# szhan227/text2protein

Measured on AMD Instinct MI355X. Metric: 6D backbone samples/sec (128-res, 1000-step), higher is better.
Workload: dtype f16; 1 GPU; cfg2: test_config.yml L=128 N=1000 chains/GPU=32 C=5 text_tokens=512 condition=none; step = 1 PC step (2 score evals + SDE updates); sample = 1000 PC steps; finite=True

## Files before the change

### include/t2p.h

```cpp
#ifndef T2P_H_
#define T2P_H_

#include <stdint.h>

#ifdef __cplusplus
extern "C" {
#endif

#define T2P_DTYPE_F32 0
#define T2P_DTYPE_BF16 1
#define T2P_DTYPE_F16 2

#define T2P_SDE_VE 0
#define T2P_SDE_VP 1

typedef struct t2p_model_config {
  int32_t num_channels;
  int32_t max_res_num;
  int32_t nf;
  int32_t num_res_blocks;
  int32_t n_ch_mult;
  int32_t ch_mult[8];
  int32_t n_attn_resolutions;
  int32_t attn_resolutions[8];
// ... 80 lines not shown
void t2p_train_destroy(t2p_trainer* t);
int t2p_train_num_params(const t2p_trainer* t);
int t2p_train_param_info(const t2p_trainer* t, int i, const char** name, int64_t shape[4], int* ndim);
int t2p_train_load_param(t2p_trainer* t, const char* name, const float* host_data, const int64_t* shape, int ndim);
int t2p_train_read(t2p_trainer* t, int which, const char* name, float* host_out);
int t2p_train_write(t2p_trainer* t, int which, const char* name, const float* host_in);
int t2p_train_set_step(t2p_trainer* t, int64_t step, int64_t adam_updates, int64_t ema_updates);
int t2p_train_get_step(const t2p_trainer* t, int64_t out3[3]);
int t2p_train_set_dropout_masks(t2p_trainer* t, const uint8_t* const* device_masks, int n);
int t2p_train_loss(t2p_trainer* t, const t2p_train_batch* batch, int backward, float* loss_host, float* score_out, void* stream);
int t2p_train_step(t2p_trainer* t, const t2p_train_batch* batch, float* loss_host, void* stream);
int t2p_train_grad_buffer(t2p_trainer* t, float** device_ptr, int64_t* n);
int t2p_train_apply(t2p_trainer* t, void* stream);
int t2p_train_eval_loss(t2p_trainer* t, const t2p_train_batch* batch, float* loss_host, void* stream);
int64_t t2p_train_device_bytes(const t2p_trainer* t);
int t2p_op_tgemm(const float* A, int64_t sAm, int64_t sAk, const float* B, int64_t sBk, int64_t sBn, float* C, int64_t ldc, int M, int N,
                 int K, int nz, int64_t sAz, int64_t sBz, int64_t sCz, float alpha, float beta, const float* bias_n, int ksplit, int conv,
                 int H, int W, int conv_C, void* stream);
int t2p_op_tgemm16(int dtype, const float* A, int64_t sAm, int64_t sAk, const float* B, int64_t sBk, int64_t sBn, float* C, int64_t ldc,
                   int M, int N, int K, int nz, int64_t sAz, int64_t sBz, int64_t sCz, float alpha, float beta, const float* bias_n, int ksplit,
                   int conv, int H, int W, int conv_C, void* stream);
int t2p_op_groupnorm_backward(const float* x, const float* dy, const float* gamma, const float* beta, int silu, int batch, int HW, int C,
                              int groups, float eps, float* dx, float* dgamma, float* dbeta, void* stream);
int t2p_op_layernorm_backward(const float* x, const float* dy, const float* gamma, int64_t rows, int C, float eps, float* dx, float* dgamma,
                              float* dbeta, void* stream);
int t2p_op_softmax_backward(const float* P, float* dP_inout, int64_t rows, int n, float scale, void* stream);
int t2p_op_geglu_backward(const float* u, const float* dy, float* du, int64_t rows, int inner, void* stream);

int t2p_op_gemm(int dtype, const void* A, int a_f32, const void* Bw, void* C, int c_f32, int M, int N, int K,
                int64_t lda, int64_t ldb, int64_t ldc, const float* bias_n, const float* residual, float alpha,
                void* stream);
int t2p_op_gemm_r16(int dtype, const void* A, int a_f32, const void* Bw, void* C, int c_f32, int M, int N, int K, int64_t lda,
                    int64_t ldb, int64_t ldc, const float* bias_n, const void* residual16, float alpha, void* stream);
int t2p_op_conv3x3(int dtype, const void* x, int a_f32, const void* w, const float* bias, float* out, int batch,
                   int H, int W, int Cin, int Cout, int upsample, void* stream);
int t2p_op_conv3x3_shortcut(int dtype, const void* a, const void* w, const float* bias, const void* x0, int CX0,
                            const void* x1, int CX1, float alpha, void* out, int c_f32, int batch, int H, int W, int C,
                            int Cout, void* stream);
int t2p_op_conv3x3_groupnorm(int dtype, const void* a, const void* w, const float* bias, const float* bias_bn, const void* residual,
                             float alpha, int upsample, int groups, const float* gamma, const float* beta, float eps, int silu,
                             void* out, int out_f32, void* normed, float* col_stats, int batch, int H, int W, int C, int Cout, void* stream);
int t2p_op_small_conv_groupnorm(int dtype, const void* a, const void* w, int64_t ldw, const void* x0, int CX0, const void* x1, int CX1,
                                const float* bias, const float* bias_bn, const void* residual, float alpha, void* out, int out_f32,
                                float* col_stats, void* normed, int groups, const float* gamma, const float* beta, float eps, int silu,
                                int batch, int H, int W, int C, int Cout, void* stream);
int t2p_op_st_entry(int dtype, const void* x, const float* col_stats, int groups, const float* gn_gamma, const float* gn_beta,
                    float gn_eps, const void* w_in, const float* b_in, const void* residual, const float* ln_gamma,
                    const float* ln_beta, float ln_eps, const void* w_2, int n2, const float* b_2, int geglu, void* t, void* out2,
                    const void* w_3, const float* b_3, const void* res3, void* y, float* y_stats, int batch, int n, int C,
                    void* stream);
int t2p_op_attn_proj(int dtype, const void* x, const float* col_stats, int groups, const float* gn_gamma, const float* gn_beta,
                     float gn_eps, const void* w_qk, const float* b_qk, const void* w_v, void* qk, void* vt, void* k_fm,
                     int64_t npad, int batch, int n, int C, void* stream);
int t2p_op_input_conv(const float* x, const float* w_tcn, const float* bias, void* out, int out_dtype, int batch, int C,
                      int H, int W, int nf, float* col_stats, void* stream);
int t2p_op_groupnorm(const float* x0, const float* x1, int C0, int C1, int batch, int H, int W, int groups,
                     const float* gamma, const float* beta, float eps, int silu, int down, void* out, int dtype,
                     void* stream);
int t2p_op_layernorm(const float* x, const float* gamma, const float* beta, void* out, int dtype, int64_t rows,
                     int C, float eps, void* stream);
int t2p_op_layernorm16(const void* x16, const float* gamma, const float* beta, void* out16, int dtype, int64_t rows, int C,
                       float eps, void* stream);
int t2p_op_softmax(const float* S, int64_t lds, void* P, int64_t ldp, int dtype, int64_t rows, int n, float scale,
                   void* stream);
int t2p_op_geglu(const float* u, void* out, int dtype, int64_t rows, int inner, void* stream);
int64_t t2p_op_attention_ws(int dtype, int batch, int heads, int nq, int nk);
// ... 47 lines not shown
```

### text2protein_amd/_lib.py

```python
from __future__ import annotations

import ctypes as C

from . import build as _build

DT_F32, DT_BF16, DT_F16 = 0, 1, 2
DTYPE_NAMES = {"f32": DT_F32, "fp32": DT_F32, "float32": DT_F32, "bf16": DT_BF16, "bfloat16": DT_BF16,
               "f16": DT_F16, "fp16": DT_F16, "float16": DT_F16}
SDE_VE, SDE_VP = 0, 1


class T2PError(RuntimeError):
    pass


class ModelConfig(C.Structure):
    _fields_ = [("num_channels", C.c_int32), ("max_res_num", C.c_int32), ("nf", C.c_int32),
                ("num_res_blocks", C.c_int32), ("n_ch_mult", C.c_int32), ("ch_mult", C.c_int32 * 8),
                ("n_attn_resolutions", C.c_int32), ("attn_resolutions", C.c_int32 * 8),
                ("n_heads", C.c_int32), ("context_dim", C.c_int32), ("num_scales", C.c_int32),
                ("sigma_min", C.c_double), ("sigma_max", C.c_double),
                ("skip_rescale", C.c_int32), ("scale_by_sigma", C.c_int32), ("compute_dtype", C.c_int32)]


# ... 28 lines not shown
    "t2p_engine_load_param": (_i, [_vp, C.c_char_p, _vp, C.POINTER(_i64), _i]),
    "t2p_engine_finalize": (_i, [_vp]),
    "t2p_engine_set_context": (_i, [_vp, _vp, _i, _i, _vp]),
    "t2p_engine_score": (_i, [_vp, _vp, _vp, _vp, _i, _vp]),
    "t2p_engine_score_ex": (_i, [_vp, _vp, _vp, _vp, _vp, _i, _vp]),
    "t2p_engine_device_bytes": (_i64, [_vp]),
    "t2p_engine_pool_reclaimed": (_i, [_vp]),
    "t2p_sampler_create": (_i, [_vp, C.POINTER(SamplerConfig), _vp, _vp, C.POINTER(_vp)]),
    "t2p_sampler_set_seed": (_i, [_vp, _u64]),
    "t2p_sampler_set_norm_allreduce": (_i, [_vp, _vp, _vp, _vp]),
    "t2p_built_with_ablation": (_i, []),
    "t2p_sampler_destroy": (None, [_vp]),
    "t2p_sampler_set_condition": (_i, [_vp, _vp, _vp]),
    "t2p_sampler_reset": (_i, [_vp, _i, _vp]),
    "t2p_sampler_step": (_i, [_vp, _vp, _vp, _vp, _vp, _vp]),
    "t2p_sampler_step_graph": (_i, [_vp, _vp, _vp, _vp]),
    "t2p_sampler_run": (_i, [_vp, _vp, _vp, _i, _i, _vp]),
    "t2p_sampler_set_vp_tables": (_i, [_vp, _vp, _vp, _vp, _vp]),
    "t2p_sampler_count_dispatches": (_i, [_vp, _vp, _vp, _vp, C.POINTER(C.c_int)]),
    "t2p_op_gemm": (_i, [_i, _vp, _i, _vp, _vp, _i, _i, _i, _i, _i64, _i64, _i64, _vp, _vp, _f, _vp]),
    "t2p_op_conv3x3_shortcut": (_i, [_i, _vp, _vp, _vp, _vp, _i, _vp, _i, _f, _vp, _i, _i, _i, _i, _i, _i, _vp]),
    "t2p_op_conv3x3_groupnorm": (_i, [_i, _vp, _vp, _vp, _vp, _vp, C.c_float, _i, _i, _vp, _vp, C.c_float, _i, _vp, _i, _vp, _vp,
                                      _i, _i, _i, _i, _i, _vp]),
    "t2p_op_attention_wide": (_i, [_i, _vp, _i64, _vp, _i64, _vp, _i64, _vp, _i, _vp, _vp, _i, _f, _vp, _i, _i, _i, _f, _vp]),
    "t2p_op_attention_wide_fm": (_i, [_i, _vp, _i64, _vp, _vp, _vp, _i, _vp, _vp, _i, _f, _vp, _i, _i, _i, _f, _vp]),
    "t2p_op_gemm_frag_major": (_i, [_i, _vp, _vp, _vp, _vp, _i, _i, _i, _i, _i, _i, _vp]),
    "t2p_op_small_conv_groupnorm": (_i, [_i, _vp, _vp, _i64, _vp, _i, _vp, _i, _vp, _vp, _vp, _f, _vp, _i, _vp, _vp, _i, _vp, _vp, _f, _i,
                                         _i, _i, _i, _i, _i, _vp]),
    "t2p_op_attn_proj": (_i, [_i, _vp, _vp, _i, _vp, _vp, _f, _vp, _vp, _vp, _vp, _vp, _vp, _i64, _i, _i, _i, _vp]),
    "t2p_op_st_entry": (_i, [_i, _vp, _vp, _i, _vp, _vp, _f, _vp, _vp, _vp, _vp, _vp, _f, _vp, _i, _vp, _i, _vp, _vp, _vp, _vp, _vp, _vp, _vp,
                             _i, _i, _i, _vp]),
    "t2p_op_input_conv": (_i, [_vp, _vp, _vp, _vp, _i, _i, _i, _i, _i, _i, _vp, _vp]),
    "t2p_op_gemm_r16": (_i, [_i, _vp, _i, _vp, _vp, _i, _i, _i, _i, _i64, _i64, _i64, _vp, _vp, _f, _vp]),
    "t2p_op_conv3x3": (_i, [_i, _vp, _i, _vp, _vp, _vp, _i, _i, _i, _i, _i, _i, _vp]),
    "t2p_op_groupnorm": (_i, [_vp, _vp, _i, _i, _i, _i, _i, _i, _vp, _vp, _f, _i, _i, _vp, _i, _vp]),
    "t2p_op_layernorm": (_i, [_vp, _vp, _vp, _vp, _i, _i64, _i, _f, _vp]),
    "t2p_op_layernorm16": (_i, [_vp, _vp, _vp, _vp, _i, _i64, _i, _f, _vp]),
    "t2p_op_softmax": (_i, [_vp, _i64, _vp, _i64, _i, _i64, _i, _f, _vp]),
    "t2p_op_geglu": (_i, [_vp, _vp, _i, _i64, _i, _vp]),
    "t2p_op_attention_ws": (_i64, [_i, _i, _i, _i, _i]),
    "t2p_op_attention_qkv": (_i, [_i, _vp, _i64, _vp, _i, _i, _i, _i, _f, _vp]),
    "t2p_op_attention": (_i, [_i, _vp, _i64, _vp, _i64, _vp, _i64, _vp, _i, _i, _i, _i, _i, _f, _vp, _vp]),
    "t2p_op_langevin": (_i, [_vp, _vp, _vp, _vp, _vp, _vp, _vp, _i, _i64, _f, _f, _vp, _vp]),
    "t2p_op_langevin_norms": (_i, [_vp, _vp, _i, _i64, _vp, _vp, _vp]),
    "t2p_op_langevin_update": (_i, [_vp, _vp, _vp, _vp, _vp, _vp, _vp, _i64, _vp, _f, _f, _f, _vp]),
    "t2p_op_apply_mask": (_i, [_vp, _vp, _vp, _i64, _vp]),
    "t2p_op_predictor": (_i, [_vp, _vp, _vp, _vp, _vp, _vp, _vp, _i64, _f, _i, _vp]),
    "t2p_op_philox_normal": (_i, [_vp, _i64, _u64, _u64, _vp]),
    "t2p_profile_begin": (_i, []),
    "t2p_debug_set": (_i, [_i, _i]),
    "t2p_op_decode_6d": (_i, [_vp, _i, _i, _i, _vp, _vp, _vp, _vp]),
    "t2p_op_embedding_gather": (_i, [_vp, _i, _vp, _vp, _i64, _i, _i, _vp, _vp]),
    "t2p_profile_end": (_i, [C.POINTER(C.c_double)]),
    "t2p_profile_dominant": (_i, [C.POINTER(C.c_double), C.c_char_p, C.c_int]),
    "t2p_profile_attention": (_i, [C.POINTER(C.c_double)]),
    "t2p_profile_shapes": (_i, [C.c_char_p, C.c_int]),
    "t2p_debug_tap": (_i, [_i, _vp, C.c_int64, C.POINTER(C.c_int64)]),
    "t2p_profile_layers_begin": (_i, []),
    "t2p_profile_layers_end": (_i, [C.c_char_p, C.c_int]),
    "t2p_op_convert": (_i, [_vp, _vp, _i, _i64, _vp]),
    "t2p_train_create": (_i, [C.POINTER(ModelConfig), C.POINTER(TrainConfig), C.POINTER(_vp)]),
    "t2p_train_destroy": (None, [_vp]),
    "t2p_train_num_params": (_i, [_vp]),
    "t2p_train_param_info": (_i, [_vp, _i, C.POINTER(C.c_char_p), C.POINTER(_i64), C.POINTER(_i)]),
    "t2p_train_load_param": (_i, [_vp, C.c_char_p, _vp, C.POINTER(_i64), _i]),
    "t2p_train_read": (_i, [_vp, _i, C.c_char_p, _vp]),
# ... 102 lines not shown
```

### text2protein_amd/build.py

```python
from __future__ import annotations

import hashlib
import os
import re
import subprocess
import sys

CSRC = os.path.join(os.path.dirname(os.path.abspath(__file__)), "csrc")
LIB = os.path.join(CSRC, "libt2p_hip.so")
LIB_ABLATION = os.path.join(CSRC, "libt2p_hip_ablation.so")
SOURCES = ["gemm.hip", "kernels.hip", "attention.hip", "smallconv.hip", "stfuse.hip", "engine.cpp", "capi.cpp",
           "train_kernels.hip", "train.cpp", "train_capi.cpp"]
GEMM_PARTS = 7
HEADERS = ["t2p_common.h", "t2p_kernels.h", "engine.h", "train_kernels.h", "train.h", os.path.join("..", "..", "include", "t2p.h")]
ARCH = "gfx950"


def _hipcc():
    for c in (os.environ.get("HIPCC"), "/opt/rocm/bin/hipcc", "hipcc"):
        if c and (os.path.isabs(c) and os.path.exists(c) or not os.path.isabs(c)):
            return c
    raise RuntimeError("hipcc not found")


STAMP = LIB + ".srchash"
FLAGS = ["-O3", "-std=c++17", "-fPIC", f"--offload-arch={ARCH}", "-Wall", "-Wno-unused-function"]
_COMPILER_ID = None


def compiler_id() -> str:
    global _COMPILER_ID
    if _COMPILER_ID is None:
        try:
            _COMPILER_ID = subprocess.run([_hipcc(), "--version"], capture_output=True, text=True, timeout=60).stdout.strip()
        except (OSError, RuntimeError, subprocess.SubprocessError):
            _COMPILER_ID = ""
    return _COMPILER_ID


def source_hash(ablation: bool = False) -> str:
    h = hashlib.sha256()
    h.update(" ".join(FLAGS + (["-DT2P_ABLATION"] if ablation else [])).encode())
    h.update(compiler_id().encode())
    for f in SOURCES + HEADERS:
        h.update(f.encode())
        with open(os.path.join(CSRC, f), "rb") as fh:
# ... 130 lines not shown
```

### text2protein_amd/csrc/capi.cpp

```cpp
#include <new>

#include "engine.h"

using namespace t2p;

#define API_BEGIN try {
#define API_END                                        \
  }                                                    \
  catch (const std::bad_alloc&) {                      \
    set_last_error("out of host memory");              \
    return T2P_ERR_STATE;                              \
  }                                                    \
  catch (const std::exception& ex) {                   \
    set_last_error(std::string("exception: ") + ex.what()); \
    return T2P_ERR_STATE;                              \
  }

namespace t2p { extern bool g_pre_conv_mfma, g_gn_apply_cols; void layer_profile_begin(); int layer_profile_end(std::string* out);
void debug_tap_set(int index, float* dst, long capacity); void debug_tap_shape(long out[4]); }
extern "C" {

const char* t2p_last_error(void) { return get_last_error(); }

int t2p_device_count(void) {
// ... 159 lines not shown
  API_END
}

int t2p_op_gemm(int dtype, const void* A, int a_f32, const void* Bw, void* C, int c_f32, int M, int N, int K, int64_t lda,
                int64_t ldb, int64_t ldc, const float* bias_n, const float* residual, float alpha, void* stream) {
  API_BEGIN
  GemmParams p;
  p.dtype = dtype; p.A0 = A; p.a_f32 = a_f32; p.C0 = K; p.lda0 = lda; p.Bw = Bw; p.ldb = ldb; p.M = M; p.N = N;
  p.bias_n = bias_n; p.R = residual; p.ldr = ldc; p.alpha = alpha; p.C = C; p.c_f32 = c_f32; p.ldc = ldc;
  return launch_gemm(p, (hipStream_t)stream);
  API_END
}

static void* g_op_ws = nullptr;
static size_t g_op_ws_bytes = 0, g_op_ws_alloc = 0;
static int attach_op_ws(GemmParams& p) {
  if (!g_op_ws_bytes) return T2P_OK;
  if (g_op_ws_alloc < g_op_ws_bytes) {
    if (g_op_ws) { T2P_HIP_CHECK(hipDeviceSynchronize()); T2P_HIP_CHECK(hipFree(g_op_ws)); g_op_ws = nullptr; g_op_ws_alloc = 0; }
    T2P_HIP_CHECK(hipMalloc(&g_op_ws, g_op_ws_bytes));
    g_op_ws_alloc = g_op_ws_bytes;
  }
  p.ws = g_op_ws; p.ws_bytes = g_op_ws_bytes;
  return T2P_OK;
}

int t2p_op_gemm_r16(int dtype, const void* A, int a_f32, const void* Bw, void* C, int c_f32, int M, int N, int K, int64_t lda,
                    int64_t ldb, int64_t ldc, const float* bias_n, const void* residual16, float alpha, void* stream) {
  API_BEGIN
  GemmParams p;
  p.dtype = dtype; p.A0 = A; p.a_f32 = a_f32; p.C0 = K; p.lda0 = lda; p.Bw = Bw; p.ldb = ldb; p.M = M; p.N = N;
  p.bias_n = bias_n; p.R = (const float*)residual16; p.r_lowp = 1; p.ldr = ldc; p.alpha = alpha; p.C = C; p.c_f32 = c_f32; p.ldc = ldc;
  T2P_TRY(attach_op_ws(p));
  return launch_gemm(p, (hipStream_t)stream);
  API_END
}

int t2p_op_conv3x3(int dtype, const void* x, int a_f32, const void* w, const float* bias, float* out, int batch, int H,
                   int W, int Cin, int Cout, int upsample, void* stream) {
  API_BEGIN
  GemmParams p;
  p.dtype = dtype; p.A0 = x; p.a_f32 = a_f32; p.C0 = Cin; p.lda0 = Cin; p.taps = 9; p.H = H; p.W = W; p.a_up = upsample;
  p.Bw = w; p.ldb = 9L * Cin; p.M = batch * H * W; p.N = Cout; p.bias_n = bias; p.rows_per_batch = H * W;
  p.C = out; p.c_f32 = 1; p.ldc = Cout;
  T2P_TRY(attach_op_ws(p));
  return launch_gemm(p, (hipStream_t)stream);
  API_END
}

int t2p_op_conv3x3_shortcut(int dtype, const void* a, const void* w, const float* bias, const void* x0, int CX0, const void* x1,
                            int CX1, float alpha, void* out, int c_f32, int batch, int H, int W, int C, int Cout, void* stream) {
  API_BEGIN
  GemmParams p;
  p.dtype = dtype; p.A0 = a; p.a_f32 = 0; p.C0 = C; p.lda0 = C; p.taps = 9; p.H = H; p.W = W;
  p.Bw = w; p.ldb = 9L * C + CX0 + CX1; p.M = batch * H * W; p.N = Cout; p.bias_n = bias; p.rows_per_batch = H * W;
  p.alpha = alpha; p.C = out; p.c_f32 = c_f32; p.ldc = Cout;
  T2P_TRY(attach_op_ws(p));
  T2P_REQUIRE(gemm_can_fuse_shortcut(p), "this convolution does not take the shortcut segment (LDS-DMA 3x3 convolutions only)");
  p.X0 = x0; p.CX0 = CX0; p.ldx0 = CX0; p.X1 = x1; p.CX1 = CX1; p.ldx1 = CX1;
  return launch_gemm(p, (hipStream_t)stream);
  API_END
}

int t2p_op_conv3x3_groupnorm(int dtype, const void* a, const void* w, const float* bias, const float* bias_bn, const void* residual,
                             float alpha, int upsample, int groups, const float* gamma, const float* beta, float eps, int silu,
                             void* out, int out_f32, void* normed, float* col_stats, int batch, int H, int W, int C, int Cout, void* stream) {
// ... 314 lines not shown
int t2p_op_apply_mask(float* x, const uint8_t* mask, const float* x_initial, int64_t n, void* stream) {
  API_BEGIN
  return launch_apply_mask(x, mask, x_initial, n, (hipStream_t)stream);
  API_END
}

int t2p_debug_set(int key, int value) {
  if (key == 10) { g_op_ws_bytes = (size_t)value << 20; return T2P_OK; }
  if (key == 11) { set_gemm_force_nsplit(value); return T2P_OK; }
  if (key == 12) { set_gemm_midsplit(value != 0); return T2P_OK; }
  if (key == 13) { g_gn_small = value != 0; return T2P_OK; }
  if (key == 14) { g_lowp_residual = value != 0; return T2P_OK; }
  if (key == 15) { set_gemm_thin_conv(value != 0); return T2P_OK; }
  if (key == 17) { g_gn_apply16 = value != 0; return T2P_OK; }
  if (key == 20) { g_layernorm16 = value != 0; return T2P_OK; }
  if (key == 21) { set_gemm_up4(value != 0); return T2P_OK; }
  if (key == 22) { set_gemm_deep_ring(value != 0); return T2P_OK; }
  if (key == 23) { set_gemm_fuse_shortcut(value != 0); return T2P_OK; }
  if (key == 25) { g_qkv_fused = value != 0; return T2P_OK; }
  if (key == 26) { t2p::g_pre_conv_mfma = value != 0; return T2P_OK; }
  if (key == 27) { t2p::g_gn_apply_cols = value != 0; return T2P_OK; }
  if (key == 28) { set_gemm_post_gn(value != 0); return T2P_OK; }
  if (key == 29) { t2p::g_attn_strip = value != 0; return T2P_OK; }
  if (key == 36) { t2p::g_small_conv = value != 0; return T2P_OK; }
  if (key == 38) { t2p::g_pre_conv_split = value != 0; return T2P_OK; }
  if (key == 39) { t2p::g_st_fuse = value != 0; return T2P_OK; }
  if (key == 40) { t2p::g_st_tail = value != 0; return T2P_OK; }
  if (key == 41) { t2p::g_small_conv_fm = value != 0; return T2P_OK; }
  if (key == 42) { t2p::g_st_ffpo = value != 0; return T2P_OK; }
  if (key == 43) { t2p::g_st_tail_rows = value; return T2P_OK; }
  if (key == 45) { t2p::g_attn_fm = value != 0; return T2P_OK; }
  if (key == 46) { t2p::g_attn_proj = value != 0; return T2P_OK; }
  if (key == 47) { set_gemm_dxs(value != 0); return T2P_OK; }
  if (key == 34) { set_gemm_a_norm(value != 0); return T2P_OK; }
  if (key == 32) { g_attn_merged = value != 0; return T2P_OK; }
  if (key == 33) { g_ffpo_merged = value != 0; return T2P_OK; }
  if (key == 30) { set_gemm_split_consts(value, 0); return T2P_OK; }
  if (key == 31) { set_gemm_split_consts(0, value); return T2P_OK; }
  if (key == 0) set_gemm_dma(value != 0);
  else if (key == 1) {
#ifndef T2P_ABLATION
    if (value & ~(128 | 256 | 4096 | 8192)) {
      set_last_error("ablation bits that skip work exist only in a -DT2P_ABLATION build");
      return T2P_ERR_INVALID;
    }
#endif
    set_gemm_debug(value);
  }
  else if (key == 2) set_gemm_geom(value);
  else if (key == 3) set_gemm_splitk(value != 0);
  else if (key == 4) g_raw_copies = value != 0;
  else if (key == 5) g_flash_attention = value != 0;
  else if (key == 6) g_fuse_gn_stats = value != 0;
  else if (key == 7) g_fuse_geglu = value != 0;
  else if (key == 8) set_gemm_ring(value);
  else if (key == 9) g_lowp_h1 = value != 0;
  else return T2P_ERR_INVALID;
  return T2P_OK;
}

#ifdef T2P_ABLATION
extern "C" int t2p_ablation_dxs_stamps(unsigned long long* out, int n) { return t2p::dxs_stamps_read(out, n); }
#endif

int t2p_built_with_ablation(void) {
#ifdef T2P_ABLATION
// ... 76 lines not shown
```

### text2protein_amd/csrc/gemm.hip

```cpp
#include <algorithm>
#include <array>
#include <cstdio>
#include <cstring>
#include <map>
#include <string>
#include <type_traits>
#include <vector>

#include "t2p_common.h"

namespace t2p {

typedef float f32x16 __attribute__((ext_vector_type(16)));
typedef __bf16 bf16x8_t __attribute__((ext_vector_type(8)));
typedef _Float16 f16x8_t __attribute__((ext_vector_type(8)));

[[maybe_unused]] static constexpr int ROWB = 144;

template <typename TC> struct VecInfo { static constexpr int VEC = 16 / (int)sizeof(TC); };

template <typename TC> __device__ inline uint4 pack16(const float* f);
template <> __device__ inline uint4 pack16<float>(const float* f) {
  uint4 r;
  r.x = __builtin_bit_cast(uint32_t, f[0]); r.y = __builtin_bit_cast(uint32_t, f[1]);
// ... 77 lines not shown
  e[2] = __builtin_bit_cast(TC, (uint16_t)u.y); e[3] = __builtin_bit_cast(TC, (uint16_t)(u.y >> 16));
  return (f32x4_res_t){to_f32(e[0]), to_f32(e[1]), to_f32(e[2]), to_f32(e[3])};
}
template <typename TC> __device__ inline float4 res_load4(const float* R, long idx, int lowp) {
  if constexpr (sizeof(TC) == 2) {
    if (lowp) {
      const f32x4_res_t v = unpack4<TC>(*(const u32x2_res_t*)((const TC*)R + idx));
      return make_float4(v[0], v[1], v[2], v[3]);
    }
  }
  return *(const float4*)(R + idx);
}

#ifndef T2P_GEMM_PART
#define T2P_GEMM_PART -1
#endif
#define T2P_PART_HOST (T2P_GEMM_PART <= 0)
#define T2P_PART_DMA (T2P_GEMM_PART != 0)

struct ProfRec { hipEvent_t a, b; double flops; int kind; const char* name; double bytes; int M = 0, N = 0, K = 0, taps = 0, z = 0; };
inline void prof_shape(ProfRec& r, const GemmParams& p) {
  r.M = p.M; r.N = p.N; r.K = p.C0 + p.C1; r.taps = p.a_up ? -p.taps : p.taps; r.z = p.nz0 * p.nz1;
  if (p.CX0 + p.CX1) r.K = r.K * 1000000 + p.CX0 + p.CX1;
}
struct DmaPlan { int geom, nsplit; };
extern bool g_prof_on;
extern std::vector<ProfRec> g_prof;
extern int g_dma_ring, g_dbg;
extern bool g_up4, g_deep_ring, g_dxs;
int num_cus();
DmaPlan dma_plan(const GemmParams& p);
int launch_splitk_reduce(const GemmParams& p, int nsplit, hipStream_t stream);
template <typename TC, int MODE> int launch_dma_mode(const GemmParams& p, hipStream_t stream);

__host__ __device__ __forceinline__ bool reg_epilogue_ok(const GemmParams& p, const int nsplit, const int dbg) {
  if (dbg & 4096) return false;
  const long c_cols = p.geglu ? p.N / 2 : p.N;
  const long c_bytes = nsplit > 1 ? (long)p.M * p.N * 4 : ((long)(p.M - 1) * p.ldc + c_cols) * (p.c_f32 ? 4 : 2);
  const int HW = p.H * p.W;
  const long r_rows = p.r_up ? (long)(p.M / HW) * (p.H >> 1) * (p.W >> 1) : (long)p.M;
  const long r_bytes = p.R ? ((r_rows - 1) * p.ldr + p.N) * (p.r_lowp ? 2 : 4) : 0;
  if ((p.N & 7) || c_bytes >= (1L << 31) || r_bytes >= (1L << 31)) return false;
  if (nsplit > 1) return true;
  if (p.geglu ? (p.ldc & 3) : (p.ldc & 7)) return false;
  if (p.R && (p.ldr & 7)) return false;
  if (p.bias_bn && ((p.ld_bn & 3) || p.rows_per_batch % 16)) return false;
  if (p.r_up && (p.W % 16 || p.rows_per_batch != HW)) return false;
  return true;
}


#if T2P_PART_HOST
template <typename TC, bool AF32, int BM, int BN>
__global__ __launch_bounds__(256) void gemm_kernel(const GemmParams p) {
  constexpr int VEC = VecInfo<TC>::VEC;
  constexpr int BK = 8 * VEC;
  constexpr int AR = BM / 32, BR = BN / 32;
  constexpr int TM = BM / 64, TN = BN / 64;
  extern __shared__ __attribute__((aligned(16))) unsigned char smem[];
  unsigned char* As = smem;
  unsigned char* Bs = smem + 2 * BM * ROWB;

  const int tid = threadIdx.x;
  const int lane = tid & 63, wave = tid >> 6;
  const int wm = wave >> 1, wn = wave & 1;
  const int lr = lane & 31, lh = lane >> 5;
// ... 1893 lines not shown
int launch_splitk_reduce(const GemmParams& p, int nsplit, hipStream_t stream) {
  return p.dtype == DT_BF16 ? launch_splitk_reduce_t<bf16_t>(p, nsplit, stream) : launch_splitk_reduce_t<f16_t>(p, nsplit, stream);
}

bool gemm_fuses_geglu(const GemmParams& p) {
  if (!dma_eligible(p) || p.nz0 * p.nz1 != 1 || p.c_f32 || p.R || p.bias_bn || p.bias_m) return false;
  if (p.N % 4 != 0 || p.ldc % 2 != 0) return false;
  return !dma_uses_splitk(p);
}

bool gemm_fuses_col_stats_lowp(const GemmParams& p) {
  GemmParams q = p;
  q.c_f32 = 1;
  return !p.c_f32 && p.dtype != DT_F32 && gemm_fuses_col_stats(q);
}

bool gemm_fuses_col_stats(const GemmParams& p) {
  if (!dma_eligible(p) || p.nz0 * p.nz1 != 1 || !p.c_f32) return false;
  if (p.N % 4 != 0 || p.ldc % 4 != 0 || (p.R && p.ldr % 4 != 0) || (p.bias_bn && p.ld_bn % 4 != 0)) return false;
  if (dma_uses_splitk(p) && !splitk_reduce_vec_ok(p)) return false;
  return p.M % 64 == 0;
}

bool gemm_writes_frag_major(const GemmParams& p) {
  if (!dma_eligible(p) || p.taps != 1 || p.c_f32 || p.geglu || p.col_stats || p.gn_out || p.r_up || p.c_nchw) return false;
  if (g_dma_ring != 2 || g_dma_geom != 0) return false;
  const DmaPlan plan = dma_plan(p);
  if (plan.geom != 1 || plan.nsplit != 1 || !reg_epilogue_ok(p, 1, 0)) return false;
  if (p.frag_col0 < 0 || p.frag_col0 % 64 != 0 || (p.N - p.frag_col0) % 32 != 0 || p.frag_ns != (p.N - p.frag_col0) / 32) return false;
  if (p.rows_per_batch > 1 ? (p.rows_per_batch % 32 != 0 || p.M % p.rows_per_batch != 0 || p.nz0 * p.nz1 != 1) : (p.M % 32 != 0 || p.nz1 != 1)) return false;
  return true;
}

#endif

#if T2P_PART_DMA
template <typename TC, int MODE, int BM, int BN, int WM, int WN, int NST, int NSTB = NST, bool MF16 = false, bool REGE = false, bool CF = false>
static int launch_dma_geom(const GemmParams& p, hipStream_t stream) {
  constexpr int smem = NST * BM * 128 + NSTB * BN * 128;
  constexpr int threads = WM * WN * 64;
  if constexpr (MF16 && !REGE && MODE != 3) {
    if (reg_epilogue_ok(p, dma_plan(p).nsplit, g_dbg)) return launch_dma_geom<TC, MODE, BM, BN, WM, WN, NST, NSTB, true, true>(p, stream);
  }
  void (*kern)(const GemmParams, const int, const int, const int);
  if constexpr (CF) kern = gemm_dma_cfrag_kernel<TC, BM, BN, WM, WN, MODE, NST, NSTB>;
  else kern = gemm_dma_kernel<TC, BM, BN, WM, WN, MODE, NST, NSTB, MF16, REGE>;
  T2P_TRY(ensure_dynamic_lds((const void*)kern, smem));
  const int Mq = MODE == 3 ? p.M / 4 : p.M;
  const int tiles_m = (Mq + BM - 1) / BM, tiles_n = (p.N + BN - 1) / BN;
  const int nsplit = MODE == 3 ? 1 : dma_plan(p).nsplit;
  dim3 grid(tiles_m * tiles_n, MODE == 3 ? (p.up_phase == 5 ? 4 : 1) : p.nz0 * p.nz1, nsplit);
  ProfRec rec;
  if (g_prof_on) {
    T2P_HIP_CHECK(hipEventCreate(&rec.a));
    T2P_HIP_CHECK(hipEventCreate(&rec.b));
    prof_shape(rec, p);
    rec.flops = MODE == 3 ? 2.0 * Mq * p.N * 4.0 * (p.C0 + p.C1) * (p.up_phase == 5 ? 4 : 1)
                          : 2.0 * p.M * p.N * ((double)p.taps * (p.C0 + p.C1) + p.CX0 + p.CX1) * p.nz0 * p.nz1;
    rec.kind = p.taps == 9 ? 0 : 1;
    static const std::string kname = std::string(CF ? "gemm_dma_cfrag_kernel<" : "gemm_dma_kernel<") + (dtype_of<TC>::value == DT_F16 ? "f16_t" : "bf16_t") + ", " +
                                     std::to_string(BM) + ", " + std::to_string(BN) + ", " + std::to_string(WM) + ", " + std::to_string(WN) +
                                     ", " + std::to_string(MODE) + ", " + std::to_string(NST) + ", " + std::to_string(NSTB) + ", " +
                                     (MF16 ? "true" : "false") + ", " + (REGE ? "true" : "false") + ">";
    rec.name = kname.c_str();
    {
      const double Ct = p.C0 + p.C1, z = (double)p.nz0 * p.nz1;
// ... 279 lines not shown
  T2P_REQUIRE((long)(p.M + 127) / 128 < 65536, "M too large for grid.y");
  if (p.X0 || p.X1 || p.CX0 || p.CX1) {
    GemmParams q = p;
    q.X0 = q.X1 = nullptr; q.CX0 = q.CX1 = 0;
    T2P_REQUIRE(p.X0 && p.CX0 > 0 && p.CX0 % 64 == 0 && p.CX1 % 64 == 0 && (p.X1 != nullptr) == (p.CX1 > 0), "shortcut segment: whole 64-channel K-tiles");
    T2P_REQUIRE(gemm_can_fuse_shortcut(q), "shortcut segment: only on the LDS-DMA 3x3 convolution (ask gemm_can_fuse_shortcut)");
    T2P_REQUIRE(((uintptr_t)p.X0 % 16) == 0 && ((uintptr_t)p.X1 % 16) == 0 && p.ldx0 % 8 == 0 && p.ldx1 % 8 == 0, "shortcut segment: 16-byte aligned rows");
    T2P_REQUIRE(((long)p.M + 512) * std::max(p.ldx0, p.ldx1) * 2 < (1L << 31) - 64 && std::max(p.ldx0, p.ldx1) * 2 < (1L << 24), "shortcut segment: 32-bit offsets");
    T2P_REQUIRE(p.ldb >= 9L * (p.C0 + p.C1) + p.CX0 + p.CX1, "shortcut segment: weight rows hold 9 (C0 + C1) + CX0 + CX1 columns");
  }
  if (p.an_stats) {
    GemmParams q = p;
    q.an_stats = nullptr;
    T2P_REQUIRE(p.an_gamma && p.an_beta && p.an_groups > 0 && p.C0 % p.an_groups == 0 && gemm_applies_a_norm(q),
                "a GroupNorm of the A operand rides only on the thin-output head convolution (ask gemm_applies_a_norm)");
  }
  if (g_thin_conv && thin_conv_eligible(p)) {
    ProfRec rec;
    if (g_prof_on) {
      T2P_HIP_CHECK(hipEventCreate(&rec.a));
      T2P_HIP_CHECK(hipEventCreate(&rec.b));
      prof_shape(rec, p);
    prof_shape(rec, p);
      rec.flops = 2.0 * p.M * p.N * 9.0 * p.C0; rec.kind = 2; rec.name = nullptr; rec.bytes = 0;
      T2P_HIP_CHECK(hipEventRecord(rec.a, stream));
    }
    const int rc = p.dtype == DT_BF16 ? launch_thin_conv<bf16_t>(p, stream) : launch_thin_conv<f16_t>(p, stream);
    if (g_prof_on) {
      T2P_HIP_CHECK(hipEventRecord(rec.b, stream));
      g_prof.push_back(rec);
    }
    return rc;
  }
  if (dma_eligible(p)) return p.dtype == DT_BF16 ? launch_dma<bf16_t>(p, stream) : launch_dma<f16_t>(p, stream);
  switch (p.dtype) {
    case DT_F32: return launch_tile<float, true>(p, stream);
    case DT_BF16: return p.a_f32 ? launch_tile<bf16_t, true>(p, stream) : launch_tile<bf16_t, false>(p, stream);
    case DT_F16: return p.a_f32 ? launch_tile<f16_t, true>(p, stream) : launch_tile<f16_t, false>(p, stream);
  }
  set_last_error("launch_gemm: unknown dtype");
  return T2P_ERR_INVALID;
}

#endif

#if T2P_GEMM_PART == -1 || T2P_GEMM_PART == 1
template int launch_dma_mode<f16_t, 0>(const GemmParams&, hipStream_t);
#endif
#if T2P_GEMM_PART == -1 || T2P_GEMM_PART == 2
template int launch_dma_mode<f16_t, 1>(const GemmParams&, hipStream_t);
#endif
#if T2P_GEMM_PART == -1 || T2P_GEMM_PART == 3
template int launch_dma_mode<f16_t, 2>(const GemmParams&, hipStream_t);
#endif
#if T2P_GEMM_PART == -1 || T2P_GEMM_PART == 4
template int launch_dma_mode<bf16_t, 0>(const GemmParams&, hipStream_t);
#endif
#if T2P_GEMM_PART == -1 || T2P_GEMM_PART == 5
template int launch_dma_mode<bf16_t, 1>(const GemmParams&, hipStream_t);
#endif
#if T2P_GEMM_PART == -1 || T2P_GEMM_PART == 6
template int launch_dma_mode<bf16_t, 2>(const GemmParams&, hipStream_t);
#endif

}
```

### text2protein_amd/csrc/t2p_common.h

```cpp
#pragma once
#include <hip/hip_runtime.h>
#include <stdint.h>
#include <string>

namespace t2p {

enum DType : int { DT_F32 = 0, DT_BF16 = 1, DT_F16 = 2 };

inline size_t dtype_size(int dt) { return dt == DT_F32 ? 4 : 2; }

struct bf16_t { uint16_t v; };
struct f16_t { _Float16 v; };

template <typename T> struct dtype_of;
template <> struct dtype_of<float> { static constexpr int value = DT_F32; };
template <> struct dtype_of<bf16_t> { static constexpr int value = DT_BF16; };
template <> struct dtype_of<f16_t> { static constexpr int value = DT_F16; };

__host__ __device__ inline uint16_t f32_to_bf16_bits(float f) {
#if defined(__HIP_DEVICE_COMPILE__)
  return __builtin_bit_cast(uint16_t, (__bf16)f);
#endif
  uint32_t u = __builtin_bit_cast(uint32_t, f);
  if ((u & 0x7fffffffu) > 0x7f800000u) return (uint16_t)((u >> 16) | 0x40);
// ... 97 lines not shown
  void* gn_out = nullptr;
  const float* an_stats = nullptr;
  const float* an_gamma = nullptr;
  const float* an_beta = nullptr;
  int an_groups = 0, an_silu = 0;
  void* c_frag = nullptr;
  int frag_col0 = 0, frag_ns = 0;
  long frag_bstride = 0;
};
bool gemm_writes_frag_major(const GemmParams& p);

int launch_gemm(const GemmParams& p, hipStream_t stream);
bool gemm_fuses_col_stats(const GemmParams& p);
bool gemm_can_fuse_shortcut(const GemmParams& p);
bool gemm_fuses_geglu(const GemmParams& p);
bool gemm_fuses_col_stats_lowp(const GemmParams& p);
bool gemm_fuses_post_gn(const GemmParams& p, int groups);
void set_gemm_post_gn(bool on);
bool gemm_applies_a_norm(const GemmParams& p);
void set_gemm_split_consts(int tiles, int target);
void set_gemm_dma(bool on);
void set_gemm_debug(int v);
void set_gemm_geom(int v);
void set_gemm_ring(int v);
void set_gemm_splitk(bool on);
void set_gemm_force_nsplit(int v);
void set_gemm_midsplit(bool on);
void set_gemm_thin_conv(bool on);
void set_gemm_a_norm(bool on);
void set_gemm_up4(bool on);
void set_gemm_deep_ring(bool on);
void set_gemm_fuse_shortcut(bool on);
void set_gemm_dxs(bool on);
#ifdef T2P_ABLATION
int dxs_stamps_read(unsigned long long* out, int n);
#endif
extern bool g_qkv_fused;
extern bool g_attn_merged, g_ffpo_merged;
extern bool g_flash_attention;
extern bool g_lowp_h1;
extern bool g_lowp_residual;
extern bool g_layernorm16;
extern bool g_gn_apply16;
extern bool g_gn_small;
extern bool g_fuse_geglu;
extern bool g_fuse_gn_stats;
extern bool g_raw_copies;
void profile_begin();
int profile_end(double out[3][3]);
int profile_dominant(double out[4], const char** name);
int profile_shapes(char* buf, int len);
bool prof_on();
void prof_attention(hipEvent_t a, hipEvent_t b, double flops);
int profile_attention(double out[3]);

}
```

Before: 0.6775 samples/s.

## Add row-resident GEMM kernel keeping full K=512 A tile in LDS

Adds a specialised GEMM path for K=512 16-bit products with large M: each workgroup loads its 128-row A slab into LDS once and sweeps all N tiles, streaming only B through a small ring. The previous tile's epilogue (bias, optional GEGLU) is interleaved with the next tile's MMA steps to hide store latency. This removes repeated A reloads across N tiles and launch fragmentation, at the cost of about 160KB of LDS per workgroup (low occupancy) and a grid of only M/128 blocks. It also exposes a fused GEGLU GEMM C entry point and a toggle to disable the new path.

```diff
diff --git a/include/t2p.h b/include/t2p.h
--- a/include/t2p.h
+++ b/include/t2p.h
@@ -136,6 +136,8 @@
                 void* stream);
 int t2p_op_gemm_r16(int dtype, const void* A, int a_f32, const void* Bw, void* C, int c_f32, int M, int N, int K, int64_t lda,
                     int64_t ldb, int64_t ldc, const float* bias_n, const void* residual16, float alpha, void* stream);
+int t2p_op_gemm_geglu(int dtype, const void* A, const void* Bw, void* C, int M, int N, int K, int64_t lda, int64_t ldb, int64_t ldc,
+                      const float* bias_n, void* stream);
 int t2p_op_conv3x3(int dtype, const void* x, int a_f32, const void* w, const float* bias, float* out, int batch,
                    int H, int W, int Cin, int Cout, int upsample, void* stream);
 int t2p_op_conv3x3_shortcut(int dtype, const void* a, const void* w, const float* bias, const void* x0, int CX0,
diff --git a/text2protein_amd/_lib.py b/text2protein_amd/_lib.py
--- a/text2protein_amd/_lib.py
+++ b/text2protein_amd/_lib.py
@@ -84,6 +84,7 @@
                              _i, _i, _i, _vp]),
     "t2p_op_input_conv": (_i, [_vp, _vp, _vp, _vp, _i, _i, _i, _i, _i, _i, _vp, _vp]),
     "t2p_op_gemm_r16": (_i, [_i, _vp, _i, _vp, _vp, _i, _i, _i, _i, _i64, _i64, _i64, _vp, _vp, _f, _vp]),
+    "t2p_op_gemm_geglu": (_i, [_i, _vp, _vp, _vp, _i, _i, _i, _i64, _i64, _i64, _vp, _vp]),
     "t2p_op_conv3x3": (_i, [_i, _vp, _i, _vp, _vp, _vp, _i, _i, _i, _i, _i, _i, _vp]),
     "t2p_op_groupnorm": (_i, [_vp, _vp, _i, _i, _i, _i, _i, _i, _vp, _vp, _f, _i, _i, _vp, _i, _vp]),
     "t2p_op_layernorm": (_i, [_vp, _vp, _vp, _vp, _i, _i64, _i, _f, _vp]),
diff --git a/text2protein_amd/build.py b/text2protein_amd/build.py
--- a/text2protein_amd/build.py
+++ b/text2protein_amd/build.py
@@ -11,7 +11,7 @@
 LIB_ABLATION = os.path.join(CSRC, "libt2p_hip_ablation.so")
 SOURCES = ["gemm.hip", "kernels.hip", "attention.hip", "smallconv.hip", "stfuse.hip", "engine.cpp", "capi.cpp",
            "train_kernels.hip", "train.cpp", "train_capi.cpp"]
-GEMM_PARTS = 7
+GEMM_PARTS = 8
 HEADERS = ["t2p_common.h", "t2p_kernels.h", "engine.h", "train_kernels.h", "train.h", os.path.join("..", "..", "include", "t2p.h")]
 ARCH = "gfx950"
 
diff --git a/text2protein_amd/csrc/capi.cpp b/text2protein_amd/csrc/capi.cpp
--- a/text2protein_amd/csrc/capi.cpp
+++ b/text2protein_amd/csrc/capi.cpp
@@ -215,6 +215,17 @@
   p.dtype = dtype; p.A0 = A; p.a_f32 = a_f32; p.C0 = K; p.lda0 = lda; p.Bw = Bw; p.ldb = ldb; p.M = M; p.N = N;
   p.bias_n = bias_n; p.R = (const float*)residual16; p.r_lowp = 1; p.ldr = ldc; p.alpha = alpha; p.C = C; p.c_f32 = c_f32; p.ldc = ldc;
   T2P_TRY(attach_op_ws(p));
+  return launch_gemm(p, (hipStream_t)stream);
+  API_END
+}
+
+int t2p_op_gemm_geglu(int dtype, const void* A, const void* Bw, void* C, int M, int N, int K, int64_t lda, int64_t ldb, int64_t ldc,
+                      const float* bias_n, void* stream) {
+  API_BEGIN
+  GemmParams p;
+  p.dtype = dtype; p.A0 = A; p.a_f32 = 0; p.C0 = K; p.lda0 = lda; p.Bw = Bw; p.ldb = ldb; p.M = M; p.N = N;
+  p.bias_n = bias_n; p.C = C; p.c_f32 = 0; p.ldc = ldc; p.geglu = 1;
+  T2P_REQUIRE(gemm_fuses_geglu(p), "this product does not take the fused GEGLU epilogue (16-bit operands on the LDS-DMA kernel, N % 4 == 0)");
   return launch_gemm(p, (hipStream_t)stream);
   API_END
 }
@@ -595,6 +606,7 @@
   if (key == 45) { t2p::g_attn_fm = value != 0; return T2P_OK; }
   if (key == 46) { t2p::g_attn_proj = value != 0; return T2P_OK; }
   if (key == 47) { set_gemm_dxs(value != 0); return T2P_OK; }
+  if (key == 48) { set_gemm_rowres(value != 0); return T2P_OK; }
   if (key == 34) { set_gemm_a_norm(value != 0); return T2P_OK; }
   if (key == 32) { g_attn_merged = value != 0; return T2P_OK; }
   if (key == 33) { g_ffpo_merged = value != 0; return T2P_OK; }
diff --git a/text2protein_amd/csrc/gemm.hip b/text2protein_amd/csrc/gemm.hip
--- a/text2protein_amd/csrc/gemm.hip
+++ b/text2protein_amd/csrc/gemm.hip
@@ -133,6 +133,7 @@
 DmaPlan dma_plan(const GemmParams& p);
 int launch_splitk_reduce(const GemmParams& p, int nsplit, hipStream_t stream);
 template <typename TC, int MODE> int launch_dma_mode(const GemmParams& p, hipStream_t stream);
+template <typename TC> int launch_rowres(const GemmParams& p, hipStream_t stream);
 
 __host__ __device__ __forceinline__ bool reg_epilogue_ok(const GemmParams& p, const int nsplit, const int dbg) {
   if (dbg & 4096) return false;
@@ -2092,6 +2093,18 @@
   return true;
 }
 
+static bool g_rowres = true;
+void set_gemm_rowres(bool on) { g_rowres = on; }
+bool gemm_rowres_eligible(const GemmParams& p) {
+  if (!g_rowres || !dma_eligible(p) || g_dma_ring != 2 || g_dma_geom != 0 || g_dbg) return false;
+  if (p.taps != 1 || p.A1 || p.C1 || p.C0 != 512 || p.nz0 * p.nz1 != 1 || p.a_up || p.X0 || p.X1) return false;
+  if (p.c_frag || p.col_stats || p.gn_out || p.c_f32 || p.bias_m || p.bias_bn || p.R || p.r_up || p.c_nchw || p.an_stats) return false;
+  if (p.M < 32768 || p.M % 128 != 0 || p.N < 1024 || p.N % 256 != 0) return false;
+  if (p.geglu && !gemm_fuses_geglu(p)) return false;
+  const DmaPlan plan = dma_plan(p);
+  return plan.geom == 1 && plan.nsplit == 1 && reg_epilogue_ok(p, 1, 0);
+}
+
 #endif
 
 #if T2P_PART_DMA
@@ -2437,6 +2450,7 @@
     }
     return rc;
   }
+  if (gemm_rowres_eligible(p)) return p.dtype == DT_BF16 ? launch_rowres<bf16_t>(p, stream) : launch_rowres<f16_t>(p, stream);
   if (dma_eligible(p)) return p.dtype == DT_BF16 ? launch_dma<bf16_t>(p, stream) : launch_dma<f16_t>(p, stream);
   switch (p.dtype) {
     case DT_F32: return launch_tile<float, true>(p, stream);
@@ -2447,6 +2461,228 @@
   return T2P_ERR_INVALID;
 }
 
+#endif
+
+#if T2P_GEMM_PART == -1 || T2P_GEMM_PART == 7
+template <typename TC, bool GEGLU>
+__global__ __launch_bounds__(256) void gemm_rowres_kernel(const GemmParams p) {
+  constexpr int BM = 128, BN = 128;
+  constexpr int ASLICE = BM * 128;
+  constexpr int BRING = 8 * ASLICE;
+  constexpr int BSTAGE = BN * 64;
+  extern __shared__ __attribute__((aligned(16))) unsigned char smem[];
+
+  const int tid = threadIdx.x;
+  const int lane = tid & 63;
+  const int wave = __builtin_amdgcn_readfirstlane(tid >> 6);
+  const int wm = wave >> 1, wn = wave & 1;
+  const int l16 = lane & 15, g4 = lane >> 4;
+  const int m0 = blockIdx.x * BM;
+  const int ntile = p.N / BN;
+
+  const __amdgpu_buffer_rsrc_t rA = make_rsrc(p.A0, (int)((((long)p.M - 1) * p.lda0 + 512) * 2));
+  const __amdgpu_buffer_rsrc_t rB = make_rsrc(p.Bw, (int)((((long)p.N - 1) * p.ldb + 512) * 2));
+  const __amdgpu_buffer_rsrc_t rBias = make_rsrc(p.bias_n ? (const void*)p.bias_n : p.A0, p.bias_n ? p.N * 4 : 0);
+  const int c_cols = GEGLU ? p.N / 2 : p.N;
+  const __amdgpu_buffer_rsrc_t rC = make_rsrc(p.C, (int)((((long)p.M - 1) * p.ldc + c_cols) * 2));
+  const unsigned ldc = (unsigned)p.ldc;
+  const unsigned ldb2 = (unsigned)(p.ldb * 2);
+  const float alpha = p.alpha;
+  const int M = p.M;
+
+  {
+    const unsigned lda2 = (unsigned)(p.lda0 * 2);
+#pragma unroll
+    for (int kt = 0; kt < 8; ++kt) {
+#pragma unroll
+      for (int j = 0; j < 4; ++j) {
+        const int r = (wave * 4 + j) * 8 + (lane >> 3);
+        const int m = m0 + r;
+        const unsigned voff = m < M ? (unsigned)m * lda2 + (unsigned)(kt * 128) + (unsigned)(((lane & 7) ^ ((r >> 1) & 7)) * 16) : DMA_OOB;
+        __builtin_amdgcn_raw_ptr_buffer_load_lds(rA, T2P_LDS_PTR(smem + kt * ASLICE + (wave * 4 + j) * 1024), 16, voff, 0, 0, 0);
+      }
+    }
+  }
+  unsigned b_off[2];
+#pragma unroll
+  for (int j = 0; j < 2; ++j) {
+    const int r = (wave * 2 + j) * 16 + (lane >> 2);
+    const int n = (r & ~63) + hperm(r & 63);
+    b_off[j] = (unsigned)n * ldb2 + (unsigned)(((lane & 3) ^ ((-(r >> 2)) & 3)) * 16);
+  }
+  auto issue_b = [&](auto SGC, auto STC, unsigned tb, bool ok) __attribute__((always_inline)) {
+    constexpr int SG = decltype(SGC)::value, ST = decltype(STC)::value;
+#pragma unroll
+    for (int j = 0; j < 2; ++j) {
+      const unsigned voff = ok ? b_off[j] + tb + (unsigned)(ST * 64) : DMA_OOB;
+      __builtin_amdgcn_raw_ptr_buffer_load_lds(rB, T2P_LDS_PTR(smem + BRING + SG * BSTAGE + (wave * 2 + j) * 1024), 16, voff, 0, 0, 0);
+    }
+  };
+  using I0 = std::integral_constant<int, 0>; using I1 = std::integral_constant<int, 1>; using I2 = std::integral_constant<int, 2>;
+  issue_b(I0{}, I0{}, 0u, true);
+  issue_b(I1{}, I1{}, 0u, true);
+  issue_b(I2{}, I2{}, 0u, true);
+
+  const unsigned lds_base = (unsigned)(unsigned long long)T2P_LDS_PTR(smem);
+  unsigned a_fo[2], b_fo;
+  {
+    const int ra = wm * 64 + l16, rb = wn * 64 + l16;
+#pragma unroll
+    for (int ks = 0; ks < 2; ++ks) a_fo[ks] = lds_base + (unsigned)(ra * 128 + (((4 * ks + g4) ^ ((ra >> 1) & 7)) << 4));
+    b_fo = lds_base + (unsigned)(BRING + rb * 64 + ((g4 ^ ((-(rb >> 2)) & 3)) << 4));
+  }
+  u32x4_t FA[2][4], FB[2][4];
+  auto read_frags = [&](auto SC) __attribute__((always_inline)) {
+    constexpr int S = decltype(SC)::value, X = S & 1;
+    const unsigned aa = a_fo[S & 1] + (unsigned)((S >> 1) * ASLICE), bb = b_fo + (unsigned)((S & 3) * BSTAGE);
+    lds_read_b128_1k<0>(FB[X][0], bb); lds_read_b128_1k<1>(FB[X][1], bb); lds_read_b128_1k<2>(FB[X][2], bb); lds_read_b128_1k<3>(FB[X][3], bb);
+    lds_read_b128_2k<0>(FA[X][0], aa); lds_read_b128_2k<1>(FA[X][1], aa); lds_read_b128_2k<2>(FA[X][2], aa); lds_read_b128_2k<3>(FA[X][3], aa);
+  };
+
+  const int col_l = wn * 64 + 8 * g4;
+  const int row_w = m0 + wm * 64;
+  float bs[16];
+  auto epi_bias = [&](int n0) __attribute__((always_inline)) {
+#pragma unroll
+    for (int h = 0; h < 2; ++h)
+#pragma unroll
+      for (int q = 0; q < 2; ++q) {
+        const f32x4_t t = __builtin_bit_cast(f32x4_t, __builtin_amdgcn_raw_buffer_load_b128(rBias, (unsigned)(n0 + col_l + 32 * h + 4 * q) * 4u, 0, 0));
+        const int k = 8 * h + 4 * q;
+        bs[k] = t[0]; bs[k + 1] = t[1]; bs[k + 2] = t[2]; bs[k + 3] = t[3];
+      }
+  };
+  auto epi_rows = [&](f32x4_t (&acc)[4][4], auto IC, int n0) __attribute__((always_inline)) {
+    constexpr int i = decltype(IC)::value;
+    const int row = row_w + 16 * i + l16;
+    float v[16];
+#pragma unroll
+    for (int j = 0; j < 4; ++j)
+#pragma unroll
+      for (int e = 0; e < 4; ++e) v[4 * j + e] = acc[i][j][e];
+    if constexpr (GEGLU) {
+      float bm = 0.f;
+      asm volatile("" : "+v"(bm));
+#pragma unroll
+      for (int k = 0; k < 16; ++k) v[k] += bm + bs[k];
+#pragma unroll
+      for (int h = 0; h < 2; ++h) {
+        const unsigned off = row < M ? ((unsigned)row * ldc + (unsigned)((n0 + col_l + 32 * h) >> 1)) * 2u : DMA_OOB;
+        const float* w = v + 8 * h;
+        __builtin_amdgcn_raw_buffer_store_b64((u32x2_t){pack2<TC>(w[0] * gelu_erf_fast(w[1]), w[2] * gelu_erf_fast(w[3])),
+                                                         pack2<TC>(w[4] * gelu_erf_fast(w[5]), w[6] * gelu_erf_fast(w[7]))}, rC, off, 0, 0);
+      }
+    } else {
+#pragma unroll
+      for (int k = 0; k < 16; ++k) v[k] += bs[k];
+      if (alpha != 1.0f) {
+#pragma unroll
+        for (int k = 0; k < 16; ++k) v[k] *= alpha;
+      }
+#pragma unroll
+      for (int h = 0; h < 2; ++h) {
+        const unsigned off = row < M ? ((unsigned)row * ldc + (unsigned)(n0 + col_l + 32 * h)) * 2u : DMA_OOB;
+        const float* w = v + 8 * h;
+        const u32x4_t packed = {pack2<TC>(w[0], w[1]), pack2<TC>(w[2], w[3]), pack2<TC>(w[4], w[5]), pack2<TC>(w[6], w[7])};
+        __builtin_amdgcn_raw_buffer_store_b128(packed, rC, off, 0, T2P_C_AUX);
+      }
+    }
+  };
+#define T2P_RR_EPI(S, HASP) ((HASP) ? ((S) == 1 ? 4 : (((S) == 4 || (S) == 6 || (S) == 8 || (S) == 10) ? 2 : 0)) : 0)
+
+  auto step = [&](auto SC, auto HC, f32x4_t (&acc)[4][4], f32x4_t (&accp)[4][4], int n0p, unsigned tb, bool more) __attribute__((always_inline)) {
+    constexpr int S = decltype(SC)::value;
+    constexpr bool HASP = decltype(HC)::value;
+    constexpr int PREV = T2P_RR_EPI((S + 15) & 15, S == 0 ? false : HASP);
+    asm volatile("s_waitcnt vmcnt(%0)" ::"n"(2 + PREV) : "memory");
+    __builtin_amdgcn_s_barrier();
+    asm volatile("" ::: "memory");
+    if constexpr (HASP && S == 1) epi_bias(n0p);
+    if constexpr (S + 3 < 16) issue_b(std::integral_constant<int, (S + 3) & 3>{}, std::integral_constant<int, S + 3>{}, tb, true);
+    else issue_b(std::integral_constant<int, (S + 3) & 3>{}, std::integral_constant<int, S + 3 - 16>{}, tb + (unsigned)BN * ldb2, more);
+    constexpr int X = S & 1;
+    if (S + 1 < 16 || more) {
+      read_frags(std::integral_constant<int, (S + 1) & 15>{});
+      asm volatile("s_waitcnt lgkmcnt(8)" : "+v"(FA[X][0]), "+v"(FA[X][1]), "+v"(FA[X][2]), "+v"(FA[X][3]), "+v"(FB[X][0]), "+v"(FB[X][1]),
+                   "+v"(FB[X][2]), "+v"(FB[X][3]));
+    } else {
+      asm volatile("s_waitcnt lgkmcnt(0)" : "+v"(FA[X][0]), "+v"(FA[X][1]), "+v"(FA[X][2]), "+v"(FA[X][3]), "+v"(FB[X][0]), "+v"(FB[X][1]),
+                   "+v"(FB[X][2]), "+v"(FB[X][3]));
+    }
+#pragma unroll
+    for (int i = 0; i < 4; ++i)
+#pragma unroll
+      for (int j = 0; j < 4; ++j) Mma16<TC>::run(FB[X][j], FA[X][i], acc[i][j]);
+    if constexpr (HASP && S == 4) {
+#pragma unroll
+      for (int k = 0; k < 16; ++k) asm volatile("" : "+v"(bs[k]));
+    }
+    if constexpr (HASP && (S == 4 || S == 6 || S == 8 || S == 10)) epi_rows(accp, std::integral_constant<int, (S - 4) / 2>{}, n0p);
+    asm volatile("" ::: "memory");
+  };
+  auto tile = [&](auto HC, f32x4_t (&acc)[4][4], f32x4_t (&accp)[4][4], int jt) __attribute__((always_inline)) {
+#pragma unroll
+    for (int i = 0; i < 4; ++i)
+#pragma unroll
+      for (int j = 0; j < 4; ++j) acc[i][j] = f32x4_t{0.f, 0.f, 0.f, 0.f};
+    const unsigned tb = (unsigned)(jt * BN) * ldb2;
+    const bool more = jt + 1 < ntile;
+    const int n0p = (jt - 1) * BN;
+#define T2P_RR_STEP(S) step(std::integral_constant<int, S>{}, HC, acc, accp, n0p, tb, more);
+    T2P_RR_STEP(0) T2P_RR_STEP(1) T2P_RR_STEP(2) T2P_RR_STEP(3) T2P_RR_STEP(4) T2P_RR_STEP(5) T2P_RR_STEP(6) T2P_RR_STEP(7)
+    T2P_RR_STEP(8) T2P_RR_STEP(9) T2P_RR_STEP(10) T2P_RR_STEP(11) T2P_RR_STEP(12) T2P_RR_STEP(13) T2P_RR_STEP(14) T2P_RR_STEP(15)
+#undef T2P_RR_STEP
+  };
+  auto epi_all = [&](f32x4_t (&acc)[4][4], int jt) __attribute__((always_inline)) {
+    epi_bias(jt * BN);
+    epi_rows(acc, I0{}, jt * BN); epi_rows(acc, I1{}, jt * BN); epi_rows(acc, I2{}, jt * BN);
+    epi_rows(acc, std::integral_constant<int, 3>{}, jt * BN);
+  };
+
+  f32x4_t acc0[4][4], acc1[4][4];
+  asm volatile("s_waitcnt vmcnt(2)" ::: "memory");
+  __builtin_amdgcn_s_barrier();
+  asm volatile("" ::: "memory");
+  read_frags(I0{});
+  tile(std::false_type{}, acc0, acc1, 0);
+  int jt = 1;
+  for (; jt + 1 < ntile; jt += 2) {
+    tile(std::true_type{}, acc1, acc0, jt);
+    tile(std::true_type{}, acc0, acc1, jt + 1);
+  }
+  if (jt < ntile) {
+    tile(std::true_type{}, acc1, acc0, jt);
+    epi_all(acc1, jt);
+  } else {
+    epi_all(acc0, ntile - 1);
+  }
+#undef T2P_RR_EPI
+}
+
+template <typename TC>
+int launch_rowres(const GemmParams& p, hipStream_t stream) {
+  constexpr int smem = 8 * 128 * 128 + 4 * 128 * 64;
+  void (*kern)(const GemmParams) = p.geglu ? gemm_rowres_kernel<TC, true> : gemm_rowres_kernel<TC, false>;
+  T2P_TRY(ensure_dynamic_lds((const void*)kern, smem));
+  ProfRec rec;
+  if (g_prof_on) {
+    T2P_HIP_CHECK(hipEventCreate(&rec.a));
+    T2P_HIP_CHECK(hipEventCreate(&rec.b));
+    prof_shape(rec, p);
+    rec.flops = 2.0 * p.M * p.N * (double)p.C0;
+    rec.kind = 1;
+    rec.name = nullptr;
+    rec.bytes = 0;
+    T2P_HIP_CHECK(hipEventRecord(rec.a, stream));
+  }
+  hipLaunchKernelGGL(kern, dim3(p.M / 128), dim3(256), smem, stream, p);
+  if (g_prof_on) {
+    T2P_HIP_CHECK(hipEventRecord(rec.b, stream));
+    g_prof.push_back(rec);
+  }
+  T2P_HIP_CHECK(hipGetLastError());
+  return T2P_OK;
+}
 #endif
 
 #if T2P_GEMM_PART == -1 || T2P_GEMM_PART == 1
@@ -2467,5 +2703,9 @@
 #if T2P_GEMM_PART == -1 || T2P_GEMM_PART == 6
 template int launch_dma_mode<bf16_t, 2>(const GemmParams&, hipStream_t);
 #endif
-
-}
+#if T2P_GEMM_PART == -1 || T2P_GEMM_PART == 7
+template int launch_rowres<f16_t>(const GemmParams&, hipStream_t);
+template int launch_rowres<bf16_t>(const GemmParams&, hipStream_t);
+#endif
+
+}
diff --git a/text2protein_amd/csrc/t2p_common.h b/text2protein_amd/csrc/t2p_common.h
--- a/text2protein_amd/csrc/t2p_common.h
+++ b/text2protein_amd/csrc/t2p_common.h
@@ -153,6 +153,8 @@
 void set_gemm_deep_ring(bool on);
 void set_gemm_fuse_shortcut(bool on);
 void set_gemm_dxs(bool on);
+void set_gemm_rowres(bool on);
+bool gemm_rowres_eligible(const GemmParams& p);
 #ifdef T2P_ABLATION
 int dxs_stamps_read(unsigned long long* out, int n);
 #endif
```

Result: slower. 0.6666 samples/s (-1.6%).
